# phonism/genrec

Measured on NVIDIA H100. Metric: hstu_train_sequences_per_sec, higher is better.
Workload: dtype bf16

## Files before the change

### genrec_b200/csrc/tc_ce.cuh

```cuda
#pragma once
#include "tc_gemm.cuh"

namespace grb {

template <int TB>
GRB_DEVINL void wgmma_m64n64k16_ss(float (&d)[32], uint64_t adesc, uint64_t bdesc, uint32_t accumulate) {
    asm volatile(
        "{\n"
        ".reg .pred p;\n"
        "setp.ne.b32 p, %34, 0;\n"
        "wgmma.mma_async.sync.aligned.m64n64k16.f32.bf16.bf16 {%0,%1,%2,%3,%4,%5,%6,%7,%8,%9,%10,%11,%12,%13,%14,%15,%16,%17,%18,%19,%20,%21,%22,%23,%24,%25,%26,%27,%28,%29,%30,%31}, %32, %33, p, 1, 1, 0, %35;\n"
        "}\n"
        : "+f"(d[0]), "+f"(d[1]), "+f"(d[2]), "+f"(d[3]), "+f"(d[4]), "+f"(d[5]), "+f"(d[6]), "+f"(d[7]), "+f"(d[8]), "+f"(d[9]), "+f"(d[10]), "+f"(d[11]), "+f"(d[12]), "+f"(d[13]), "+f"(d[14]), "+f"(d[15]), "+f"(d[16]), "+f"(d[17]), "+f"(d[18]), "+f"(d[19]), "+f"(d[20]), "+f"(d[21]), "+f"(d[22]), "+f"(d[23]), "+f"(d[24]), "+f"(d[25]), "+f"(d[26]), "+f"(d[27]), "+f"(d[28]), "+f"(d[29]), "+f"(d[30]), "+f"(d[31])
        : "l"(adesc), "l"(bdesc), "r"(accumulate), "n"(TB));
}
template <int TB>
GRB_DEVINL void wgmma_m64n64k16_rs(float (&d)[32], const uint32_t (&a)[4], uint64_t bdesc, uint32_t accumulate) {
    asm volatile(
        "{\n"
        ".reg .pred p;\n"
        "setp.ne.b32 p, %37, 0;\n"
        "wgmma.mma_async.sync.aligned.m64n64k16.f32.bf16.bf16 {%0,%1,%2,%3,%4,%5,%6,%7,%8,%9,%10,%11,%12,%13,%14,%15,%16,%17,%18,%19,%20,%21,%22,%23,%24,%25,%26,%27,%28,%29,%30,%31}, {%32,%33,%34,%35}, %36, p, 1, 1, %38;\n"
        "}\n"
        : "+f"(d[0]), "+f"(d[1]), "+f"(d[2]), "+f"(d[3]), "+f"(d[4]), "+f"(d[5]), "+f"(d[6]), "+f"(d[7]), "+f"(d[8]), "+f"(d[9]), "+f"(d[10]), "+f"(d[11]), "+f"(d[12]), "+f"(d[13]), "+f"(d[14]), "+f"(d[15]), "+f"(d[16]), "+f"(d[17]), "+f"(d[18]), "+f"(d[19]), "+f"(d[20]), "+f"(d[21]), "+f"(d[22]), "+f"(d[23]), "+f"(d[24]), "+f"(d[25]), "+f"(d[26]), "+f"(d[27]), "+f"(d[28]), "+f"(d[29]), "+f"(d[30]), "+f"(d[31])
        : "r"(a[0]), "r"(a[1]), "r"(a[2]), "r"(a[3]), "l"(bdesc), "r"(accumulate), "n"(TB));
}
template <int TB>
GRB_DEVINL void wgmma_m64n128k16_rs(float (&d)[64], const uint32_t (&a)[4], uint64_t bdesc, uint32_t accumulate) {
    asm volatile(
        "{\n"
        ".reg .pred p;\n"
        "setp.ne.b32 p, %69, 0;\n"
        "wgmma.mma_async.sync.aligned.m64n128k16.f32.bf16.bf16 {%0,%1,%2,%3,%4,%5,%6,%7,%8,%9,%10,%11,%12,%13,%14,%15,%16,%17,%18,%19,%20,%21,%22,%23,%24,%25,%26,%27,%28,%29,%30,%31,%32,%33,%34,%35,%36,%37,%38,%39,%40,%41,%42,%43,%44,%45,%46,%47,%48,%49,%50,%51,%52,%53,%54,%55,%56,%57,%58,%59,%60,%61,%62,%63}, {%64,%65,%66,%67}, %68, p, 1, 1, %70;\n"
        "}\n"
        : "+f"(d[0]), "+f"(d[1]), "+f"(d[2]), "+f"(d[3]), "+f"(d[4]), "+f"(d[5]), "+f"(d[6]), "+f"(d[7]), "+f"(d[8]), "+f"(d[9]), "+f"(d[10]), "+f"(d[11]), "+f"(d[12]), "+f"(d[13]), "+f"(d[14]), "+f"(d[15]), "+f"(d[16]), "+f"(d[17]), "+f"(d[18]), "+f"(d[19]), "+f"(d[20]), "+f"(d[21]), "+f"(d[22]), "+f"(d[23]), "+f"(d[24]), "+f"(d[25]), "+f"(d[26]), "+f"(d[27]), "+f"(d[28]), "+f"(d[29]), "+f"(d[30]), "+f"(d[31]), "+f"(d[32]), "+f"(d[33]), "+f"(d[34]), "+f"(d[35]), "+f"(d[36]), "+f"(d[37]), "+f"(d[38]), "+f"(d[39]), "+f"(d[40]), "+f"(d[41]), "+f"(d[42]), "+f"(d[43]), "+f"(d[44]), "+f"(d[45]), "+f"(d[46]), "+f"(d[47]), "+f"(d[48]), "+f"(d[49]), "+f"(d[50]), "+f"(d[51]), "+f"(d[52]), "+f"(d[53]), "+f"(d[54]), "+f"(d[55]), "+f"(d[56]), "+f"(d[57]), "+f"(d[58]), "+f"(d[59]), "+f"(d[60]), "+f"(d[61]), "+f"(d[62]), "+f"(d[63])
        : "r"(a[0]), "r"(a[1]), "r"(a[2]), "r"(a[3]), "l"(bdesc), "r"(accumulate), "n"(TB));
}

template <int D>
GRB_DEVINL void wgmma_rs_d(float (&d)[D / 2], const uint32_t (&a)[4], uint64_t bdesc) {
    if constexpr (D == 64) wgmma_m64n64k16_rs<1>(d, a, bdesc, 1u);
    else wgmma_m64n128k16_rs<1>(d, a, bdesc, 1u);
}

constexpr int CE_THREADS = 384;
constexpr int CE_STAGES = 4;
constexpr float CE_L2E = 1.4426950408889634f;

struct CeArgs {
    const long long* tg;
    const float* inv_count;
    int T, C;
    float* dx;
    float* shift;
    float* row_loss;
    float* dtable;
};

template <int D>
struct CeSmem {
    static constexpr int XB = D / 64;
    static constexpr int ROW_TILE = XB * 128 * 128;
    static constexpr int CLS_TILE = XB * 64 * 128;
    static constexpr int ROWS_BYTES = ROW_TILE + CE_STAGES * CLS_TILE + 1024 + 256;
    static constexpr int TABLE_BYTES = CLS_TILE + CE_STAGES * CLS_TILE + 1024 + 256;
};

template <int D>
GRB_DEVINL void ce_scores(float (&S)[32], uint32_t a_addr, int a_box, uint32_t b_addr) {
    wgmma_fence();
#pragma unroll
    for (int kk = 0; kk < D / 16; ++kk)
        wgmma_m64n64k16_ss<0>(S, wgmma_desc(a_addr + (kk >> 2) * a_box + (kk & 3) * 32, 16, 1024),
                              wgmma_desc(b_addr + (kk >> 2) * 8192 + (kk & 3) * 32, 16, 1024), kk > 0 ? 1u : 0u);
    wgmma_commit();
    wgmma_wait<0>();
}
template <int D>
GRB_DEVINL void ce_accumulate(float (&acc)[D / 2], const float (&G)[32], uint32_t b_addr) {
    uint32_t a[4][4];
#pragma unroll
    for (int kk = 0; kk < 4; ++kk) {
        a[kk][0] = pack_bf16(G[8 * kk], G[8 * kk + 1]);
        a[kk][1] = pack_bf16(G[8 * kk + 2], G[8 * kk + 3]);
        a[kk][2] = pack_bf16(G[8 * kk + 4], G[8 * kk + 5]);
        a[kk][3] = pack_bf16(G[8 * kk + 6], G[8 * kk + 7]);
    }
    wgmma_fence();
#pragma unroll
    for (int kk = 0; kk < 4; ++kk) wgmma_rs_d<D>(acc, a[kk], wgmma_desc(b_addr + kk * 2048, 8192, 1024));
    wgmma_commit();
    wgmma_wait<0>();
}

template <int D>
__global__ void __launch_bounds__(CE_THREADS, 1)
    ce_rows_kernel(const __grid_constant__ CUtensorMap tmX, const __grid_constant__ CUtensorMap tmE, CeArgs a) {
    using SM = CeSmem<D>;
    extern __shared__ unsigned char ce_smem_raw[];
    unsigned char* base = ce_smem_raw + ((1024u - (smem_u32(ce_smem_raw) & 1023u)) & 1023u);
    unsigned char* sX = base;
    unsigned char* sE = base + SM::ROW_TILE;
    uint64_t* bars = reinterpret_cast<uint64_t*>(sE + CE_STAGES * SM::CLS_TILE);
    uint64_t* full = bars;
    uint64_t* empty = bars + CE_STAGES;
    uint64_t* xfull = bars + 2 * CE_STAGES;
    const int warp = threadIdx.x >> 5, lane = threadIdx.x & 31;
    const int row0 = blockIdx.x * 128;
    if (threadIdx.x == 0) {
        tma_prefetch_desc(&tmX);
        tma_prefetch_desc(&tmE);
        for (int s = 0; s < CE_STAGES; ++s) { mbar_init(&full[s], 1); mbar_init(&empty[s], 2); }
        mbar_init(xfull, 1);
        fence_barrier_init();
    }
    __syncthreads();
    pdl_wait();
    const int ntile = (a.C + 63) / 64;
    const int sweeps = a.dx ? 2 : 1;

    if (warp < 4) {
        if (warp == 0 && lane == 0) {
            mbar_expect_tx(xfull, SM::ROW_TILE);
            for (int b = 0; b < SM::XB; ++b) tma_load_2d(sX + b * 16384, &tmX, b * 64, row0, xfull);
            int stage = 0;
            uint32_t phase = 0;
            for (int sw = 0; sw < sweeps; ++sw)
                for (int j = 0; j < ntile; ++j) {
                    mbar_wait(&empty[stage], phase ^ 1);
                    mbar_expect_tx(&full[stage], SM::CLS_TILE);
                    for (int b = 0; b < SM::XB; ++b) tma_load_2d(sE + stage * SM::CLS_TILE + b * 8192, &tmE, b * 64, j * 64, &full[stage]);
                    if (++stage == CE_STAGES) { stage = 0; phase ^= 1; }
                }
        }
        return;
    }
    const int g = (warp >> 2) - 1, w = warp & 3, q = lane & 3;
    const bool leader = (threadIdx.x & 127) == 0;
    int row[2], tgt[2];
    float ic[2];
    const float inv = *a.inv_count;
#pragma unroll
    for (int i = 0; i < 2; ++i) {
        row[i] = row0 + 64 * g + 16 * w + (lane >> 2) + 8 * i;
        tgt[i] = row[i] < a.T ? (int)a.tg[row[i]] : 0;
        ic[i] = tgt[i] != 0 ? inv : 0.f;
    }
    mbar_wait(xfull, 0);
    const uint32_t xa = smem_u32(sX) + g * 8192;
    int stage = 0;
    uint32_t phase = 0;
    float m[2] = {-INFINITY, -INFINITY}, s[2] = {0.f, 0.f}, tl[2] = {0.f, 0.f};
    for (int j = 0; j < ntile; ++j) {
        mbar_wait(&full[stage], phase);
        float S[32];
        ce_scores<D>(S, xa, 16384, smem_u32(sE + stage * SM::CLS_TILE));
        if (leader) mbar_arrive(&empty[stage]);
        if (++stage == CE_STAGES) { stage = 0; phase ^= 1; }
#pragma unroll
        for (int i = 0; i < 2; ++i) {
            float mx = -INFINITY;
#pragma unroll
            for (int jj = 0; jj < 8; ++jj)
#pragma unroll
                for (int c = 0; c < 2; ++c) {
                    const int col = j * 64 + 8 * jj + 2 * q + c;
                    float& v = S[jj * 4 + i * 2 + c];
                    if (col >= a.C) v = -INFINITY;
                    if (col == tgt[i]) tl[i] = v;
                    mx = fmaxf(mx, v);
                }
            mx = fmaxf(mx, __shfl_xor_sync(0xffffffffu, mx, 1));
            mx = fmaxf(mx, __shfl_xor_sync(0xffffffffu, mx, 2));
            const float mn = fmaxf(m[i], mx);
            float acc = s[i] * ex2_fast((m[i] - mn) * CE_L2E);
#pragma unroll
            for (int jj = 0; jj < 8; ++jj)
#pragma unroll
                for (int c = 0; c < 2; ++c) acc += ex2_fast((S[jj * 4 + i * 2 + c] - mn) * CE_L2E);
            s[i] = acc;
            m[i] = mn;
        }
    }
    float shift[2];
#pragma unroll
    for (int i = 0; i < 2; ++i) {
        s[i] += __shfl_xor_sync(0xffffffffu, s[i], 1);
        s[i] += __shfl_xor_sync(0xffffffffu, s[i], 2);
        tl[i] += __shfl_xor_sync(0xffffffffu, tl[i], 1);
        tl[i] += __shfl_xor_sync(0xffffffffu, tl[i], 2);
        shift[i] = m[i] * CE_L2E + __log2f(s[i]);
        if (q == 0 && row[i] < a.T) {
            a.row_loss[row[i]] = tgt[i] != 0 ? (m[i] + __logf(s[i]) - tl[i]) * ic[i] : 0.f;
            a.shift[row[i]] = shift[i];
        }
    }
    if (!a.dx) return;
    float dx[D / 2];
#pragma unroll
    for (int k = 0; k < D / 2; ++k) dx[k] = 0.f;
    for (int j = 0; j < ntile; ++j) {
        mbar_wait(&full[stage], phase);
        float S[32];
        const uint32_t e_addr = smem_u32(sE + stage * SM::CLS_TILE);
        ce_scores<D>(S, xa, 16384, e_addr);
#pragma unroll
        for (int jj = 0; jj < 8; ++jj)
#pragma unroll
            for (int i = 0; i < 2; ++i)
#pragma unroll
                for (int c = 0; c < 2; ++c) {
                    const int col = j * 64 + 8 * jj + 2 * q + c;
                    float& v = S[jj * 4 + i * 2 + c];
                    float gv = col < a.C ? ex2_fast(v * CE_L2E - shift[i]) * ic[i] : 0.f;
                    if (col == tgt[i]) gv -= ic[i];
                    v = gv;
                }
        ce_accumulate<D>(dx, S, e_addr);
        if (leader) mbar_arrive(&empty[stage]);
        if (++stage == CE_STAGES) { stage = 0; phase ^= 1; }
    }
#pragma unroll
    for (int jj = 0; jj < D / 8; ++jj)
#pragma unroll
        for (int i = 0; i < 2; ++i)
            if (row[i] < a.T)
                *reinterpret_cast<float2*>(a.dx + (size_t)row[i] * D + 8 * jj + 2 * q) = make_float2(dx[jj * 4 + i * 2], dx[jj * 4 + i * 2 + 1]);
}

template <int D>
__global__ void __launch_bounds__(CE_THREADS, 1)
    ce_table_kernel(const __grid_constant__ CUtensorMap tmX, const __grid_constant__ CUtensorMap tmE, CeArgs a) {
    using SM = CeSmem<D>;
    extern __shared__ unsigned char ce_smem_raw[];
    unsigned char* base = ce_smem_raw + ((1024u - (smem_u32(ce_smem_raw) & 1023u)) & 1023u);
    unsigned char* sE = base;
    unsigned char* sX = base + SM::CLS_TILE;
    uint64_t* bars = reinterpret_cast<uint64_t*>(sX + CE_STAGES * SM::CLS_TILE);
    uint64_t* full = bars;
    uint64_t* empty = bars + CE_STAGES;
    uint64_t* efull = bars + 2 * CE_STAGES;
    const int warp = threadIdx.x >> 5, lane = threadIdx.x & 31;
    const int cls0 = blockIdx.x * 64;
    if (threadIdx.x == 0) {
        tma_prefetch_desc(&tmX);
        tma_prefetch_desc(&tmE);
        for (int s = 0; s < CE_STAGES; ++s) { mbar_init(&full[s], 1); mbar_init(&empty[s], 1); }
        mbar_init(efull, 1);
        fence_barrier_init();
    }
    __syncthreads();
    pdl_wait();
    const int ntt = (a.T + 63) / 64;
    const int g = (warp >> 2) - 1, w = warp & 3, q = lane & 3;
    float acc[D / 2];
    if (warp < 4) {
        if (warp == 0 && lane == 0) {
            mbar_expect_tx(efull, SM::CLS_TILE);
            for (int b = 0; b < SM::XB; ++b) tma_load_2d(sE + b * 8192, &tmE, b * 64, cls0, efull);
            for (int tt = 0; tt < ntt; ++tt) {
                const int stage = tt % CE_STAGES;
                mbar_wait(&empty[stage], ((tt / CE_STAGES) & 1) ^ 1);
                mbar_expect_tx(&full[stage], SM::CLS_TILE);
                for (int b = 0; b < SM::XB; ++b) tma_load_2d(sX + stage * SM::CLS_TILE + b * 8192, &tmX, b * 64, tt * 64, &full[stage]);
            }
        }
    } else {
        const bool leader = (threadIdx.x & 127) == 0;
        int cls[2];
#pragma unroll
        for (int i = 0; i < 2; ++i) cls[i] = cls0 + 16 * w + (lane >> 2) + 8 * i;
        const float inv = *a.inv_count;
#pragma unroll
        for (int k = 0; k < D / 2; ++k) acc[k] = 0.f;
        mbar_wait(efull, 0);
        const uint32_t ea = smem_u32(sE) + 0;
        for (int tt = g; tt < ntt; tt += 2) {
            const int stage = tt % CE_STAGES;
            float sh[16], icc[16];
            int tg[16];
#pragma unroll
            for (int jj = 0; jj < 8; ++jj)
#pragma unroll
                for (int c = 0; c < 2; ++c) {
                    const int t = tt * 64 + 8 * jj + 2 * q + c;
                    const bool ok = t < a.T;
                    tg[jj * 2 + c] = ok ? (int)a.tg[t] : 0;
                    sh[jj * 2 + c] = ok ? a.shift[t] : 0.f;
                    icc[jj * 2 + c] = tg[jj * 2 + c] != 0 ? inv : 0.f;
                }
            mbar_wait(&full[stage], (tt / CE_STAGES) & 1);
            const uint32_t x_addr = smem_u32(sX + stage * SM::CLS_TILE);
            float S[32];
            ce_scores<D>(S, ea + 0, 8192, x_addr);
#pragma unroll
            for (int jj = 0; jj < 8; ++jj)
#pragma unroll
                for (int i = 0; i < 2; ++i)
#pragma unroll
                    for (int c = 0; c < 2; ++c) {
                        float& v = S[jj * 4 + i * 2 + c];
                        const int k = jj * 2 + c;
                        float gv = ex2_fast(v * CE_L2E - sh[k]) * icc[k];
                        if (cls[i] == tg[k]) gv -= icc[k];
                        v = gv;
                    }
            ce_accumulate<D>(acc, S, x_addr);
            if (leader) mbar_arrive(&empty[stage]);
        }
    }
    float* red = reinterpret_cast<float*>(sX);
    asm volatile("bar.sync 1, 384;" ::: "memory");
    if (g == 1) {
#pragma unroll
        for (int k = 0; k < D / 2; ++k) red[(size_t)k * 128 + (threadIdx.x & 127)] = acc[k];
    }
    asm volatile("bar.sync 1, 384;" ::: "memory");
    if (g == 0) {
#pragma unroll
        for (int jj = 0; jj < D / 8; ++jj)
#pragma unroll
            for (int i = 0; i < 2; ++i) {
                const int c = cls0 + 16 * w + (lane >> 2) + 8 * i;
                const int k = jj * 4 + i * 2;
                const float v0 = acc[k] + red[(size_t)k * 128 + (threadIdx.x & 127)];
                const float v1 = acc[k + 1] + red[(size_t)(k + 1) * 128 + (threadIdx.x & 127)];
                if (c < a.C) {
                    float* dst = a.dtable + (size_t)c * D + 8 * jj + 2 * q;
                    atomicAdd(dst, v0);
                    atomicAdd(dst + 1, v1);
                }
            }
    }
}

template <int D>
inline cudaError_t ce_set_smem() {
    static bool attr_set[64] = {false};
    int dev = 0;
    cudaGetDevice(&dev);
    if (attr_set[dev & 63]) return cudaSuccess;
    cudaError_t e = cudaFuncSetAttribute(ce_rows_kernel<D>, cudaFuncAttributeMaxDynamicSharedMemorySize, CeSmem<D>::ROWS_BYTES);
    if (e == cudaSuccess) e = cudaFuncSetAttribute(ce_table_kernel<D>, cudaFuncAttributeMaxDynamicSharedMemorySize, CeSmem<D>::TABLE_BYTES);
    if (e == cudaSuccess) attr_set[dev & 63] = true;
    return e;
}
template <int D>
inline cudaError_t launch_tc_ce(const bf16* xf, const bf16* table, const CeArgs& a, cudaStream_t st) {
    CUtensorMap tmX, tmE;
    if (!make_tmap_bf16(&tmX, xf, a.T, D, D, 64, 128) || !make_tmap_bf16(&tmE, table, a.C, D, D, 64, 64)) return cudaErrorInvalidValue;
    cudaError_t e = ce_set_smem<D>();
    if (e != cudaSuccess) return e;
    launch_k(ce_rows_kernel<D>, (a.T + 127) / 128, CE_THREADS, CeSmem<D>::ROWS_BYTES, st, tmX, tmE, a);
    return cudaGetLastError();
}
template <int D>
inline cudaError_t launch_ce_table(const bf16* xf, const bf16* table, const CeArgs& a, cudaStream_t st) {
    CUtensorMap tmX, tmE;
    if (!make_tmap_bf16(&tmX, xf, a.T, D, D, 64, 64) || !make_tmap_bf16(&tmE, table, a.C, D, D, 64, 64)) return cudaErrorInvalidValue;
    cudaError_t e = ce_set_smem<D>();
    if (e != cudaSuccess) return e;
    launch_k(ce_table_kernel<D>, (a.C + 63) / 64, CE_THREADS, CeSmem<D>::TABLE_BYTES, st, tmX, tmE, a);
    return cudaGetLastError();
}

}
```

Measured before the change: 35940.

## Double-buffer CE score wgmma to overlap next tile with softmax stats

Splits score computation into an async issue step and restructures the forward cross-entropy loop to ping-pong between two score accumulators. The next tile's wgmma is issued before waiting on the previous one, so the online max/sum-exp work overlaps tensor-core execution. Releasing a stage is deferred until its scores are consumed, which raises register pressure (two 32-float accumulators plus a temporary copy) and holds pipeline stages longer.

```diff
diff --git a/genrec_b200/csrc/tc_ce.cuh b/genrec_b200/csrc/tc_ce.cuh
--- a/genrec_b200/csrc/tc_ce.cuh
+++ b/genrec_b200/csrc/tc_ce.cuh
@@ -75,6 +75,15 @@
                               wgmma_desc(b_addr + (kk >> 2) * 8192 + (kk & 3) * 32, 16, 1024), kk > 0 ? 1u : 0u);
     wgmma_commit();
     wgmma_wait<0>();
+}
+template <int D>
+GRB_DEVINL void ce_scores_issue(float (&S)[32], uint32_t a_addr, int a_box, uint32_t b_addr) {
+    wgmma_fence();
+#pragma unroll
+    for (int kk = 0; kk < D / 16; ++kk)
+        wgmma_m64n64k16_ss<0>(S, wgmma_desc(a_addr + (kk >> 2) * a_box + (kk & 3) * 32, 16, 1024),
+                              wgmma_desc(b_addr + (kk >> 2) * 8192 + (kk & 3) * 32, 16, 1024), kk > 0 ? 1u : 0u);
+    wgmma_commit();
 }
 template <int D>
 GRB_DEVINL void ce_accumulate(float (&acc)[D / 2], const float (&G)[32], uint32_t b_addr) {
@@ -151,12 +160,8 @@
     int stage = 0;
     uint32_t phase = 0;
     float m[2] = {-INFINITY, -INFINITY}, s[2] = {0.f, 0.f}, tl[2] = {0.f, 0.f};
-    for (int j = 0; j < ntile; ++j) {
-        mbar_wait(&full[stage], phase);
-        float S[32];
-        ce_scores<D>(S, xa, 16384, smem_u32(sE + stage * SM::CLS_TILE));
-        if (leader) mbar_arrive(&empty[stage]);
-        if (++stage == CE_STAGES) { stage = 0; phase ^= 1; }
+    auto stats = [&](const float (&S)[32], int j) {
+        float v[32];
 #pragma unroll
         for (int i = 0; i < 2; ++i) {
             float mx = -INFINITY;
@@ -164,11 +169,10 @@
             for (int jj = 0; jj < 8; ++jj)
 #pragma unroll
                 for (int c = 0; c < 2; ++c) {
-                    const int col = j * 64 + 8 * jj + 2 * q + c;
-                    float& v = S[jj * 4 + i * 2 + c];
-                    if (col >= a.C) v = -INFINITY;
-                    if (col == tgt[i]) tl[i] = v;
-                    mx = fmaxf(mx, v);
+                    const int col = j * 64 + 8 * jj + 2 * q + c, k = jj * 4 + i * 2 + c;
+                    v[k] = col >= a.C ? -INFINITY : S[k];
+                    if (col == tgt[i]) tl[i] = v[k];
+                    mx = fmaxf(mx, v[k]);
                 }
             mx = fmaxf(mx, __shfl_xor_sync(0xffffffffu, mx, 1));
             mx = fmaxf(mx, __shfl_xor_sync(0xffffffffu, mx, 2));
@@ -177,9 +181,41 @@
 #pragma unroll
             for (int jj = 0; jj < 8; ++jj)
 #pragma unroll
-                for (int c = 0; c < 2; ++c) acc += ex2_fast((S[jj * 4 + i * 2 + c] - mn) * CE_L2E);
+                for (int c = 0; c < 2; ++c) acc += ex2_fast((v[jj * 4 + i * 2 + c] - mn) * CE_L2E);
             s[i] = acc;
             m[i] = mn;
+        }
+    };
+    auto issue = [&](float (&S)[32]) {
+        mbar_wait(&full[stage], phase);
+        ce_scores_issue<D>(S, xa, 16384, smem_u32(sE + stage * SM::CLS_TILE));
+        if (++stage == CE_STAGES) { stage = 0; phase ^= 1; }
+    };
+    auto done = [&](const float (&S)[32], int j, int behind) {
+        if (leader) mbar_arrive(&empty[(stage + CE_STAGES - behind) % CE_STAGES]);
+        stats(S, j);
+    };
+    {
+        float Sa[32], Sb[32];
+        issue(Sa);
+        int j = 0;
+        for (; j + 2 < ntile; j += 2) {
+            issue(Sb);
+            wgmma_wait<1>();
+            done(Sa, j, 2);
+            issue(Sa);
+            wgmma_wait<1>();
+            done(Sb, j + 1, 2);
+        }
+        if (j + 1 < ntile) {
+            issue(Sb);
+            wgmma_wait<1>();
+            done(Sa, j, 2);
+            wgmma_wait<0>();
+            done(Sb, j + 1, 1);
+        } else {
+            wgmma_wait<0>();
+            done(Sa, j, 1);
         }
     }
     float shift[2];
```

Result: no change. 36110, median of 6 (+0.5%).

## Split CE rows kernel into two sweeps with double-buffered async wgmma

Applied to the files above, without the earlier changes.

Splits the cross-entropy rows kernel into two launches, one computing the softmax statistics and one computing dx, each a template specialization. Score wgmmas are double-buffered so the next tile's scores are issued while the current tile is processed, and the dx accumulate wgmma is left asynchronous. Pipeline depth grows to six stages, and setmaxnreg moves registers from the producer warps to the consumer warps. The aim is to hide tensor-core latency behind the exp/softmax math, at the cost of re-reading the X tile and an extra launch, with shift passed between launches through global memory.

```diff
diff --git a/genrec_b200/csrc/tc_ce.cuh b/genrec_b200/csrc/tc_ce.cuh
--- a/genrec_b200/csrc/tc_ce.cuh
+++ b/genrec_b200/csrc/tc_ce.cuh
@@ -1,4 +1,6 @@
 #pragma once
+#include <type_traits>
+
 #include "tc_gemm.cuh"
 
 namespace grb {
@@ -45,6 +47,7 @@
 
 constexpr int CE_THREADS = 384;
 constexpr int CE_STAGES = 4;
+constexpr int CE_ROW_STAGES = 6;
 constexpr float CE_L2E = 1.4426950408889634f;
 
 struct CeArgs {
@@ -62,7 +65,7 @@
     static constexpr int XB = D / 64;
     static constexpr int ROW_TILE = XB * 128 * 128;
     static constexpr int CLS_TILE = XB * 64 * 128;
-    static constexpr int ROWS_BYTES = ROW_TILE + CE_STAGES * CLS_TILE + 1024 + 256;
+    static constexpr int ROWS_BYTES = ROW_TILE + CE_ROW_STAGES * CLS_TILE + 1024 + 256;
     static constexpr int TABLE_BYTES = CLS_TILE + CE_STAGES * CLS_TILE + 1024 + 256;
 };
 
@@ -93,53 +96,93 @@
     wgmma_wait<0>();
 }
 
-template <int D>
+template <int N>
+GRB_DEVINL void wgmma_fence_regs(float (&r)[N]) {
+#pragma unroll
+    for (int i = 0; i < N; ++i) asm volatile("" : "+f"(r[i])::"memory");
+}
+template <int D>
+GRB_DEVINL void ce_scores_issue(float (&S)[32], uint32_t a_addr, uint32_t b_addr) {
+    wgmma_fence_regs(S);
+    wgmma_fence();
+#pragma unroll
+    for (int kk = 0; kk < D / 16; ++kk)
+        wgmma_m64n64k16_ss<0>(S, wgmma_desc(a_addr + (kk >> 2) * 16384 + (kk & 3) * 32, 16, 1024),
+                              wgmma_desc(b_addr + (kk >> 2) * 8192 + (kk & 3) * 32, 16, 1024), kk > 0 ? 1u : 0u);
+    wgmma_commit();
+    wgmma_fence_regs(S);
+}
+GRB_DEVINL void ce_pack_g(uint32_t (&a)[4][4], const float (&G)[32]) {
+#pragma unroll
+    for (int kk = 0; kk < 4; ++kk) {
+        a[kk][0] = pack_bf16(G[8 * kk], G[8 * kk + 1]);
+        a[kk][1] = pack_bf16(G[8 * kk + 2], G[8 * kk + 3]);
+        a[kk][2] = pack_bf16(G[8 * kk + 4], G[8 * kk + 5]);
+        a[kk][3] = pack_bf16(G[8 * kk + 6], G[8 * kk + 7]);
+    }
+}
+template <int D>
+GRB_DEVINL void ce_accumulate_issue(float (&acc)[D / 2], const uint32_t (&a)[4][4], uint32_t b_addr, uint32_t accumulate) {
+    wgmma_fence_regs(acc);
+    wgmma_fence();
+#pragma unroll
+    for (int kk = 0; kk < 4; ++kk) {
+        if constexpr (D == 64) wgmma_m64n64k16_rs<1>(acc, a[kk], wgmma_desc(b_addr + kk * 2048, 8192, 1024), kk > 0 ? 1u : accumulate);
+        else wgmma_m64n128k16_rs<1>(acc, a[kk], wgmma_desc(b_addr + kk * 2048, 8192, 1024), kk > 0 ? 1u : accumulate);
+    }
+    wgmma_commit();
+    wgmma_fence_regs(acc);
+}
+
+template <int D, int SWEEP>
 __global__ void __launch_bounds__(CE_THREADS, 1)
     ce_rows_kernel(const __grid_constant__ CUtensorMap tmX, const __grid_constant__ CUtensorMap tmE, CeArgs a) {
     using SM = CeSmem<D>;
+    constexpr int NS = CE_ROW_STAGES;
     extern __shared__ unsigned char ce_smem_raw[];
     unsigned char* base = ce_smem_raw + ((1024u - (smem_u32(ce_smem_raw) & 1023u)) & 1023u);
     unsigned char* sX = base;
     unsigned char* sE = base + SM::ROW_TILE;
-    uint64_t* bars = reinterpret_cast<uint64_t*>(sE + CE_STAGES * SM::CLS_TILE);
+    uint64_t* bars = reinterpret_cast<uint64_t*>(sE + NS * SM::CLS_TILE);
     uint64_t* full = bars;
-    uint64_t* empty = bars + CE_STAGES;
-    uint64_t* xfull = bars + 2 * CE_STAGES;
+    uint64_t* empty = bars + NS;
+    uint64_t* xfull = bars + 2 * NS;
     const int warp = threadIdx.x >> 5, lane = threadIdx.x & 31;
     const int row0 = blockIdx.x * 128;
     if (threadIdx.x == 0) {
         tma_prefetch_desc(&tmX);
         tma_prefetch_desc(&tmE);
-        for (int s = 0; s < CE_STAGES; ++s) { mbar_init(&full[s], 1); mbar_init(&empty[s], 2); }
+        for (int s = 0; s < NS; ++s) { mbar_init(&full[s], 1); mbar_init(&empty[s], 2); }
         mbar_init(xfull, 1);
         fence_barrier_init();
     }
     __syncthreads();
     pdl_wait();
     const int ntile = (a.C + 63) / 64;
-    const int sweeps = a.dx ? 2 : 1;
 
     if (warp < 4) {
+        asm volatile("setmaxnreg.dec.sync.aligned.u32 24;");
         if (warp == 0 && lane == 0) {
             mbar_expect_tx(xfull, SM::ROW_TILE);
             for (int b = 0; b < SM::XB; ++b) tma_load_2d(sX + b * 16384, &tmX, b * 64, row0, xfull);
-            int stage = 0;
-            uint32_t phase = 0;
-            for (int sw = 0; sw < sweeps; ++sw)
-                for (int j = 0; j < ntile; ++j) {
-                    mbar_wait(&empty[stage], phase ^ 1);
-                    mbar_expect_tx(&full[stage], SM::CLS_TILE);
-                    for (int b = 0; b < SM::XB; ++b) tma_load_2d(sE + stage * SM::CLS_TILE + b * 8192, &tmE, b * 64, j * 64, &full[stage]);
-                    if (++stage == CE_STAGES) { stage = 0; phase ^= 1; }
-                }
+            for (int j = 0; j < ntile; ++j) {
+                const int stage = j % NS;
+                mbar_wait(&empty[stage], ((j / NS) & 1) ^ 1);
+                mbar_expect_tx(&full[stage], SM::CLS_TILE);
+                for (int b = 0; b < SM::XB; ++b) tma_load_2d(sE + stage * SM::CLS_TILE + b * 8192, &tmE, b * 64, j * 64, &full[stage]);
+            }
         }
         return;
     }
+    asm volatile("setmaxnreg.inc.sync.aligned.u32 240;");
     const int g = (warp >> 2) - 1, w = warp & 3, q = lane & 3;
     const bool leader = (threadIdx.x & 127) == 0;
+    const float inv = *a.inv_count;
+    auto e_addr = [&](int j) { return smem_u32(sE + (j % NS) * SM::CLS_TILE); };
+    auto wait_full = [&](int j) { mbar_wait(&full[j % NS], (j / NS) & 1); };
+    auto release = [&](int j) { if (leader) mbar_arrive(&empty[j % NS]); };
     int row[2], tgt[2];
     float ic[2];
-    const float inv = *a.inv_count;
 #pragma unroll
     for (int i = 0; i < 2; ++i) {
         row[i] = row0 + 64 * g + 16 * w + (lane >> 2) + 8 * i;
@@ -148,84 +191,107 @@
     }
     mbar_wait(xfull, 0);
     const uint32_t xa = smem_u32(sX) + g * 8192;
-    int stage = 0;
-    uint32_t phase = 0;
-    float m[2] = {-INFINITY, -INFINITY}, s[2] = {0.f, 0.f}, tl[2] = {0.f, 0.f};
-    for (int j = 0; j < ntile; ++j) {
-        mbar_wait(&full[stage], phase);
-        float S[32];
-        ce_scores<D>(S, xa, 16384, smem_u32(sE + stage * SM::CLS_TILE));
-        if (leader) mbar_arrive(&empty[stage]);
-        if (++stage == CE_STAGES) { stage = 0; phase ^= 1; }
+    float S0[32], S1[32];
+    using Yes = std::true_type;
+    using No = std::false_type;
+    wait_full(0);
+    ce_scores_issue<D>(S0, xa, e_addr(0));
+    auto run = [&](auto step) {
+        int j = 0;
+        for (; j + 2 < ntile; j += 2) {
+            step(No{}, S0, S1, j);
+            step(No{}, S1, S0, j + 1);
+        }
+        if (j + 1 < ntile) {
+            step(No{}, S0, S1, j);
+            step(Yes{}, S1, S0, j + 1);
+        } else {
+            step(Yes{}, S0, S1, j);
+        }
+    };
+    if constexpr (SWEEP == 1) {
+        float m[2] = {-INFINITY, -INFINITY}, s[2] = {0.f, 0.f}, tl[2] = {0.f, 0.f};
+        run([&](auto last, float (&Sc)[32], float (&Sn)[32], int j) {
+            if constexpr (!decltype(last)::value) {
+                wait_full(j + 1);
+                ce_scores_issue<D>(Sn, xa, e_addr(j + 1));
+                wgmma_wait<1>();
+            } else {
+                wgmma_wait<0>();
+            }
+            release(j);
+#pragma unroll
+            for (int i = 0; i < 2; ++i) {
+                float mx = -INFINITY, v[16];
+#pragma unroll
+                for (int jj = 0; jj < 8; ++jj)
+#pragma unroll
+                    for (int c = 0; c < 2; ++c) {
+                        const int col = j * 64 + 8 * jj + 2 * q + c;
+                        v[jj * 2 + c] = col < a.C ? Sc[jj * 4 + i * 2 + c] : -INFINITY;
+                        if (col == tgt[i]) tl[i] = v[jj * 2 + c];
+                        mx = fmaxf(mx, v[jj * 2 + c]);
+                    }
+                mx = fmaxf(mx, __shfl_xor_sync(0xffffffffu, mx, 1));
+                mx = fmaxf(mx, __shfl_xor_sync(0xffffffffu, mx, 2));
+                const float mn = fmaxf(m[i], mx);
+                float acc = s[i] * ex2_fast((m[i] - mn) * CE_L2E);
+#pragma unroll
+                for (int k = 0; k < 16; ++k) acc += ex2_fast((v[k] - mn) * CE_L2E);
+                s[i] = acc;
+                m[i] = mn;
+            }
+        });
 #pragma unroll
         for (int i = 0; i < 2; ++i) {
-            float mx = -INFINITY;
+            s[i] += __shfl_xor_sync(0xffffffffu, s[i], 1);
+            s[i] += __shfl_xor_sync(0xffffffffu, s[i], 2);
+            tl[i] += __shfl_xor_sync(0xffffffffu, tl[i], 1);
+            tl[i] += __shfl_xor_sync(0xffffffffu, tl[i], 2);
+            if (q == 0 && row[i] < a.T) {
+                a.row_loss[row[i]] = tgt[i] != 0 ? (m[i] + __logf(s[i]) - tl[i]) * ic[i] : 0.f;
+                a.shift[row[i]] = m[i] * CE_L2E + __log2f(s[i]);
+            }
+        }
+    } else {
+        float shift[2];
+#pragma unroll
+        for (int i = 0; i < 2; ++i) shift[i] = row[i] < a.T ? a.shift[row[i]] : 0.f;
+        float dx[D / 2];
+        uint32_t A[4][4];
+        run([&](auto last, float (&Sc)[32], float (&Sn)[32], int j) {
+            if constexpr (!decltype(last)::value) {
+                wait_full(j + 1);
+                ce_scores_issue<D>(Sn, xa, e_addr(j + 1));
+                wgmma_wait<1>();
+            } else {
+                wgmma_wait<0>();
+            }
+            if (j > 0) release(j - 1);
+            float G[32];
 #pragma unroll
             for (int jj = 0; jj < 8; ++jj)
 #pragma unroll
-                for (int c = 0; c < 2; ++c) {
-                    const int col = j * 64 + 8 * jj + 2 * q + c;
-                    float& v = S[jj * 4 + i * 2 + c];
-                    if (col >= a.C) v = -INFINITY;
-                    if (col == tgt[i]) tl[i] = v;
-                    mx = fmaxf(mx, v);
-                }
-            mx = fmaxf(mx, __shfl_xor_sync(0xffffffffu, mx, 1));
-            mx = fmaxf(mx, __shfl_xor_sync(0xffffffffu, mx, 2));
-            const float mn = fmaxf(m[i], mx);
-            float acc = s[i] * ex2_fast((m[i] - mn) * CE_L2E);
-#pragma unroll
-            for (int jj = 0; jj < 8; ++jj)
-#pragma unroll
-                for (int c = 0; c < 2; ++c) acc += ex2_fast((S[jj * 4 + i * 2 + c] - mn) * CE_L2E);
-            s[i] = acc;
-            m[i] = mn;
-        }
-    }
-    float shift[2];
-#pragma unroll
-    for (int i = 0; i < 2; ++i) {
-        s[i] += __shfl_xor_sync(0xffffffffu, s[i], 1);
-        s[i] += __shfl_xor_sync(0xffffffffu, s[i], 2);
-        tl[i] += __shfl_xor_sync(0xffffffffu, tl[i], 1);
-        tl[i] += __shfl_xor_sync(0xffffffffu, tl[i], 2);
-        shift[i] = m[i] * CE_L2E + __log2f(s[i]);
-        if (q == 0 && row[i] < a.T) {
-            a.row_loss[row[i]] = tgt[i] != 0 ? (m[i] + __logf(s[i]) - tl[i]) * ic[i] : 0.f;
-            a.shift[row[i]] = shift[i];
-        }
-    }
-    if (!a.dx) return;
-    float dx[D / 2];
-#pragma unroll
-    for (int k = 0; k < D / 2; ++k) dx[k] = 0.f;
-    for (int j = 0; j < ntile; ++j) {
-        mbar_wait(&full[stage], phase);
-        float S[32];
-        const uint32_t e_addr = smem_u32(sE + stage * SM::CLS_TILE);
-        ce_scores<D>(S, xa, 16384, e_addr);
-#pragma unroll
-        for (int jj = 0; jj < 8; ++jj)
+                for (int i = 0; i < 2; ++i)
+#pragma unroll
+                    for (int c = 0; c < 2; ++c) {
+                        const int col = j * 64 + 8 * jj + 2 * q + c;
+                        float gv = col < a.C ? ex2_fast(Sc[jj * 4 + i * 2 + c] * CE_L2E - shift[i]) * ic[i] : 0.f;
+                        if (col == tgt[i]) gv -= ic[i];
+                        G[jj * 4 + i * 2 + c] = gv;
+                    }
+            ce_pack_g(A, G);
+            ce_accumulate_issue<D>(dx, A, e_addr(j), j > 0 ? 1u : 0u);
+        });
+        wgmma_wait<0>();
+        release(ntile - 1);
+#pragma unroll
+        for (int jj = 0; jj < D / 8; ++jj)
 #pragma unroll
             for (int i = 0; i < 2; ++i)
-#pragma unroll
-                for (int c = 0; c < 2; ++c) {
-                    const int col = j * 64 + 8 * jj + 2 * q + c;
-                    float& v = S[jj * 4 + i * 2 + c];
-                    float gv = col < a.C ? ex2_fast(v * CE_L2E - shift[i]) * ic[i] : 0.f;
-                    if (col == tgt[i]) gv -= ic[i];
-                    v = gv;
-                }
-        ce_accumulate<D>(dx, S, e_addr);
-        if (leader) mbar_arrive(&empty[stage]);
-        if (++stage == CE_STAGES) { stage = 0; phase ^= 1; }
-    }
-#pragma unroll
-    for (int jj = 0; jj < D / 8; ++jj)
-#pragma unroll
-        for (int i = 0; i < 2; ++i)
-            if (row[i] < a.T)
-                *reinterpret_cast<float2*>(a.dx + (size_t)row[i] * D + 8 * jj + 2 * q) = make_float2(dx[jj * 4 + i * 2], dx[jj * 4 + i * 2 + 1]);
+                if (row[i] < a.T)
+                    *reinterpret_cast<float2*>(a.dx + (size_t)row[i] * D + 8 * jj + 2 * q) = make_float2(dx[jj * 4 + i * 2], dx[jj * 4 + i * 2 + 1]);
+    }
 }
 
 template <int D>
@@ -340,7 +406,8 @@
     int dev = 0;
     cudaGetDevice(&dev);
     if (attr_set[dev & 63]) return cudaSuccess;
-    cudaError_t e = cudaFuncSetAttribute(ce_rows_kernel<D>, cudaFuncAttributeMaxDynamicSharedMemorySize, CeSmem<D>::ROWS_BYTES);
+    cudaError_t e = cudaFuncSetAttribute(ce_rows_kernel<D, 1>, cudaFuncAttributeMaxDynamicSharedMemorySize, CeSmem<D>::ROWS_BYTES);
+    if (e == cudaSuccess) e = cudaFuncSetAttribute(ce_rows_kernel<D, 2>, cudaFuncAttributeMaxDynamicSharedMemorySize, CeSmem<D>::ROWS_BYTES);
     if (e == cudaSuccess) e = cudaFuncSetAttribute(ce_table_kernel<D>, cudaFuncAttributeMaxDynamicSharedMemorySize, CeSmem<D>::TABLE_BYTES);
     if (e == cudaSuccess) attr_set[dev & 63] = true;
     return e;
@@ -351,7 +418,11 @@
     if (!make_tmap_bf16(&tmX, xf, a.T, D, D, 64, 128) || !make_tmap_bf16(&tmE, table, a.C, D, D, 64, 64)) return cudaErrorInvalidValue;
     cudaError_t e = ce_set_smem<D>();
     if (e != cudaSuccess) return e;
-    launch_k(ce_rows_kernel<D>, (a.T + 127) / 128, CE_THREADS, CeSmem<D>::ROWS_BYTES, st, tmX, tmE, a);
+    const int nrt = (a.T + 127) / 128;
+    launch_k(ce_rows_kernel<D, 1>, nrt, CE_THREADS, CeSmem<D>::ROWS_BYTES, st, tmX, tmE, a);
+    if (a.dx) {
+        launch_k(ce_rows_kernel<D, 2>, nrt, CE_THREADS, CeSmem<D>::ROWS_BYTES, st, tmX, tmE, a);
+    }
     return cudaGetLastError();
 }
 template <int D>
```

Measured after the change: 35600 before, 36170 after (median of 6 runs). About the same (+1.6%).
